# ecmwf/anemoi-core

Measured on AMD Instinct MI355X. Metric: forward nodes*channels/sec on O96 GraphTransformer, higher is better.
Workload: dtype bf16; 1 GPU; AnemoiModelEncProcDec forward, O96 data grid (40320 nodes, 84 vars x 2 steps) -> icosphere res 5 hidden mesh (10242 nodes, 81840 edges), GraphTransformer processor 16 layers x 512 ch x 16 heads, enc 62912 / dec 120960 edges, batch 1; parallelism=single GPU, hip_graph=True, graph_equals_eager=True, graph_segments=1

## Files before the change

### anemoi_core_amd/_lib.py

```python
from __future__ import annotations

import ctypes as C
import os
import threading

ABI_VERSION = 26
LIB_PATH = os.path.join(os.path.dirname(os.path.abspath(__file__)), "lib", "libanemoi_hip.so")

F32, BF16, F16 = 0, 1, 2
ACT_NONE, ACT_GELU = 0, 1
E_INVALID, E_UNSUPPORTED, E_LAUNCH = -1, -2, -3

_p, _i64, _i32, _f = C.c_void_p, C.c_int64, C.c_int32, C.c_float



class LinearPlan(C.Structure):
    _fields_ = [(name, _i32) for name in ("kernel", "tile_m", "tile_n", "pingpong", "stage_k", "mi", "wr", "kg", "stages", "epi", "main_rows",
                                          "tail_rows", "ln_tail_begin")]


class AttentionPlan(C.Structure):
    _fields_ = [(name, _i32) for name in ("route", "vec", "lph", "fe_pad", "kv_adjacent", "lds_bytes")] + \
               [(name, C.c_uint32) for name in ("grid_dst", "grid_src", "grid_wgrad")]
# ... 73 lines not shown
    "anemoi_glu_fwd": ([_p, _i64, _p, _i64, _i32, _i32, _i32, C.c_int, _p], C.c_int),
    "anemoi_glu_bwd": ([_p, _i64, _p, _i64, _p, _i64, _i32, _i32, _i32, C.c_int, _p], C.c_int),
    "anemoi_gather_rows": ([_p, _i64, _p, _p, _i64, _i32, _i32, C.c_int, _p], C.c_int),
    "anemoi_peer_alloc": ([C.POINTER(_p), _i64, _i32], C.c_int),
    "anemoi_peer_free": ([_p], C.c_int),
    "anemoi_peer_export": ([_p, _p], C.c_int),
    "anemoi_peer_open": ([_p, C.POINTER(_p)], C.c_int),
    "anemoi_peer_close": ([_p], C.c_int),
    "anemoi_gt_chain_rows_per_tile": ([_i32], C.c_int),
    "anemoi_chain_plan": ([C.POINTER(ChainProblem), C.POINTER(ChainPlan)], C.c_int),
    "anemoi_gt_chain2_fwd": ([_p, C.c_int, _p], C.c_int),
    "anemoi_gt_rowchain_fwd": ([_p, C.c_int, _p], C.c_int),
    "anemoi_gt_rowchain_panels_fwd": ([_p, C.c_int32, C.c_int32, C.c_int, _p], C.c_int),
    "anemoi_gt_embed_fold_fwd": ([_p, C.c_int, _p], C.c_int),
    "anemoi_gt_chain2_side_fwd": ([_p, _p, C.c_int32, C.c_int32, C.c_int32, C.c_int, _p], C.c_int),
    "anemoi_gt_cluster_chain_fwd": ([_p, C.c_int, _p], C.c_int),
    "anemoi_gt_cluster_chain_workspace_bytes": ([], _i64),
    "anemoi_gnn_edge_chain_fwd": ([_p, _i64, _p, _i64, _p, _p, _i64, _p, _p, _p, _p, _p, _p, _p, _p, _p, _f, _p, _i64, _i32, _i32, C.c_int, _p], C.c_int),
    "anemoi_gnn_mlp_chain_fwd": ([_p, _i64, _i32, _p, _p, _p, _p, _p, _p, _p, _p, _f, _p, _i64, _p, _i64, _i32, _i32, C.c_int, _p], C.c_int),
    "anemoi_gnn_node_chain_segsum_fwd": ([_p, _i64, _p, _i64, _p, _p, _p, _p, _p, _p, _p, _p, _p, _f, _p, _i64, _p, _p, _i32, _p, _i64, _i32, _i32,
                                          C.c_int, _p], C.c_int),
    "anemoi_gnn_node_chain_fwd": ([_p, _i64, _p, _i64, _p, _p, _p, _p, _p, _p, _p, _p, _f, _p, _i64, _p, _p, _i32, _p, _i64, _i32, _i32, C.c_int, _p], C.c_int),
    "anemoi_peer_exchange_rows": ([_p, _i64, _p, _p, _i32, _i32, _i32, _p, _p, _i64, _p], C.c_int),
    "anemoi_window_attention_fwd": ([_p, _i64, _p, _i64, _p, _i64, _p, _i64, _p, _i32, _i32, _i32, _i32, _i32, _f, _f, _p, C.c_int, _p], C.c_int),
    "anemoi_window_attention_bwd": ([_p, _i64, _p, _i64, _p, _i64, _p, _i64, _p, _i64, _p, _p, _i64, _p, _i64, _p, _i64, _p, _i32, _i32, _i32, _i32,
                                     _i32, _f, _f, _p, _i32, C.c_int, _p], C.c_int),
    "anemoi_window_attention_plan": ([_i32, _i32, _i32, _i32, C.c_int, _i32, _i32, C.POINTER(WindowAttentionPlan), C.POINTER(_i32), _i32], C.c_int),
    "anemoi_sparse_project_fwd": ([_p, _i64, _i64, _i32, _i64, _i32, _i32, _p, _p, _p, _p, _p, _p, _p, _i64, _i64, _i32, _i32, _i32, C.c_int, C.c_int, _p], C.c_int),
    "anemoi_sht_plan": ([_i32, _i32, C.POINTER(_i32), _i32, _i32, C.POINTER(ShtPlan)], C.c_int),
    "anemoi_sht_fwd": ([_p, _i64, _i64, _p, _i32, _i32, _p, _i32, _i32, _i32, _p, _p, _p, _p, _i64, _p], C.c_int),
# ... 76 lines not shown
```

### anemoi_core_amd/build.py

```python
from __future__ import annotations

import os
import shutil
import subprocess
import sys
from concurrent.futures import ThreadPoolExecutor

PKG = os.path.dirname(os.path.abspath(__file__))
REPO = os.path.dirname(PKG)
CSRC = os.path.join(PKG, "csrc")
LIBDIR = os.path.join(PKG, "lib")
LIBPATH = os.path.join(LIBDIR, "libanemoi_hip.so")
EXT_PATH = os.path.join(LIBDIR, "libanemoi_torch.so")
INCLUDE = os.path.join(REPO, "include")

SOURCES = ["lib.cpp", "gt_attention.hip", "gt_attention_bwd.hip", "rowwise.hip", "model_edge.hip", "rowwise_bwd.hip", "linear.hip", "wgrad.hip", "peer.hip", "gt_chain2.hip", "gt_chain2_side.hip", "gt_rowchain.hip", "gt_embed_fold.hip", "gt_cluster_chain.hip", "gnn_chain.hip", "window_attention.hip", "window_attention_bwd.hip", "sparse_project.hip", "sht.hip", "transport.hip", "transport_bwd.hip"]
EXPERIMENT_SOURCES = ["experiments/gt_chain.hip", "experiments/gnn_chain2.hip"]
EXP_LIBPATH = os.path.join(LIBDIR, "libanemoi_hip_exp.so")
ARCH = "gfx950"


def _hipcc() -> str:
    for cand in (os.environ.get("HIPCC"), shutil.which("hipcc"), "/opt/rocm/bin/hipcc"):
        if cand and os.path.exists(cand):
            return cand
    raise RuntimeError("hipcc not found (need ROCm >= 7.0)")


def _newer(target: str, deps: list[str]) -> bool:
    if not os.path.exists(target):
        return False
# ... 83 lines not shown
```

### anemoi_core_amd/csrc/chain_host.h

```cpp
#pragma once
#include "chain_plan.h"
#include "common.h"

namespace anemoi {

inline const ChainSwitches& chain_switches() {
  static const ChainSwitches sw = [] {
    ChainSwitches s;
    s.chain_rows = env_int(getenv("ANEMOI_CHAIN_ROWS"), 0, 0, kGnnEdgeRows);
    s.gnn_node_rows = ANEMOI_EXPERIMENT_ENV("ANEMOI_GNN_NODE_ROWS", 0, 0, kPanel);
    s.even_grid = ANEMOI_EXPERIMENT_ENV("ANEMOI_CHAIN2_EVEN_GRID", 1, 0, 1) != 0;
    s.max_grid = ANEMOI_EXPERIMENT_ENV("ANEMOI_CHAIN2_MAX_GRID", kChipCus, 8, kChipCus);
    s.timeline_built = kExperiments;
    return s;
  }();
  return sw;
}

inline int chain_refused(const char* who, const ChainProblem& q, const ChainPlan& p) {
  if (p.status != ANEMOI_OK)
    set_error("%s: %s (n_rows=%d in_features=%d hidden=%d q_out_features=%d rows_per_tile=%d dtype=%d)", who, p.why, q.n_rows, q.in_features, q.hidden,
              q.q_out_features, q.rows_per_tile, (int)q.dtype);
  return p.status;
}

inline bool al16(const void* q) { return (reinterpret_cast<uintptr_t>(q) & 15) == 0; }

#define ANEMOI_CHAIN_LAUNCH(kernel, max_lds, plan, stream, args)                                                                                     \
// ... 8 lines not shown
```

### anemoi_core_amd/csrc/chain_plan.h

```cpp
#pragma once
#include <stdint.h>

#include "anemoi_hip.h"

namespace anemoi {

constexpr int kXcds = 8, kCusPerXcd = 32;
constexpr int kChipCus = kXcds * kCusPerXcd;
constexpr int kCh = 512;
constexpr int kPanel = 48;
constexpr int kGnnEdgeRows = 64;
constexpr int kClusterSize = 4;
constexpr int kVecMaxElems = 6144;
constexpr int kVecMaxElemsTl = 5120;
constexpr int kRowChainMaxQ = 4 * kCh;
constexpr int kRowChainPipeMaxIn = 256;
constexpr int kEfRows = 80, kEfThreads = 256;
constexpr int kEfMaxIn = 256, kEfMaxQ = 2048;

constexpr int kRowBytes = kCh * 2;
constexpr int kBufBytes = kPanel * kRowBytes;
constexpr int kRedOff = 3 * kBufBytes;
constexpr int vec_off(int waves) { return kRedOff + kPanel * waves * 2 * 4; }
constexpr int kChainSmem = vec_off(8);
constexpr int kChain2Lds = vec_off(4) + kVecMaxElems * 2;
constexpr int kChain2TlLds = vec_off(4) + kVecMaxElemsTl * 2 + 8 * 48 * 8;
constexpr int kRowChainLds = vec_off(8) + (kCh + kRowChainMaxQ) * 2;
constexpr int kRowChainPipeLds = vec_off(4) + (kCh + kRowChainMaxQ) * 2;
constexpr int max_of(int a, int b) { return a > b ? a : b; }
constexpr int kChain2SideLds = max_of(kChain2Lds, max_of(kRowChainLds, kRowChainPipeLds));
constexpr int kClusterLds = vec_off(8) + (2 * kCh + 4 * kCh + kRowChainMaxQ) * 2;
constexpr int kGnnEdgeLds = 2 * kGnnEdgeRows * kRowBytes + kGnnEdgeRows * 8 * 2 * 4;
constexpr int ef_lds(int qc) { return kEfRows * 512 + kEfRows * 4 * 2 * 4 + 4 * 16 * 256 + (kCh + 3 * kCh * qc) * 4; }

struct ChainSwitches {
  int chain_rows = 0;
  int gnn_node_rows = 0;
  bool even_grid = true;
  int max_grid = kChipCus;
  bool timeline_built = false;
};

enum class ChainKind : int32_t { BlockTail = 0, BlockTailSide, ClusterTail, RowChain, RowChainPanels, EmbedFold, GnnEdge, GnnMlp, GnnNode };
enum class ChainKernel : int32_t {
  None = 0,
  Chain2Full,
  Chain2Part,
  Chain2TlFull,
  Chain2TlPart,
  Chain2Side,
  Cluster,
  RowChainSingle,
  RowChainPipe,
  EmbedFold,
  GnnEdge,
  GnnMlp,
  GnnNode,
};
constexpr const char* chain_kernel_name(ChainKernel k) {
  switch (k) {
    case ChainKernel::None: return "none";
    case ChainKernel::Chain2Full: return "gt_chain2_kernel";
    case ChainKernel::Chain2Part: return "gt_chain2_kernel<false,true>";
    case ChainKernel::Chain2TlFull: return "gt_chain2_kernel<true>";
    case ChainKernel::Chain2TlPart: return "gt_chain2_kernel<true,true>";
    case ChainKernel::Chain2Side: return "gt_chain2_kernel<false,true,true>";
    case ChainKernel::Cluster: return "gt_cluster_chain_kernel";
    case ChainKernel::RowChainSingle: return "gt_rowchain_kernel";
    case ChainKernel::RowChainPipe: return "gt_rowchain_pipe_kernel";
    case ChainKernel::EmbedFold: return "gt_embed_fold_kernel";
    case ChainKernel::GnnEdge: return "gnn_edge_chain_kernel";
    case ChainKernel::GnnMlp: return "gnn_edge_chain_kernel<true>";
    case ChainKernel::GnnNode: return "gnn_node_chain_kernel";
  }
  return "?";
}

struct ChainProblem {
  ChainKind kind = ChainKind::BlockTail;
  int n_rows = 0;
  int in_features = 0;
  int hidden = 0;
  int q_out_features = 0;
  int rows_per_tile = 0;
  anemoi_dtype_t dtype = ANEMOI_BF16;
  bool timeline = false;
  int first_panel = 0, panels = 0;
  int side_rows = 0, side_in_features = 0, side_q_out_features = 0, side_rows_per_tile = 0, side_cap = 0;
// ... 165 lines not shown
    case ChainKind::GnnMlp:
    case ChainKind::GnnNode: {
      if (!bits16) return refuse(ANEMOI_E_INVALID, "16-bit model dtypes only");
      if (q.n_rows < 0) return refuse(ANEMOI_E_INVALID, "n_rows must not be negative");
      if (q.kind == ChainKind::GnnMlp && !(q.in_features >= 128 && q.in_features <= kCh && q.in_features % 128 == 0))
        return refuse(ANEMOI_E_INVALID, "in_features is the zero-padded width: 128, 256, 384 or 512");
      if (q.n_rows == 0) return ChainPlan{};
      const bool node = q.kind == ChainKind::GnnNode;
      int rpt = gnn_rows_per_tile(q.n_rows, node ? kPanel : kGnnEdgeRows, sw.chain_rows);
      if (node && sw.gnn_node_rows > 0) rpt = sw.gnn_node_rows;
      set_panels(p, q.n_rows, rpt, -1);
      p.kernel = node ? ChainKernel::GnnNode : q.kind == ChainKind::GnnMlp ? ChainKernel::GnnMlp : ChainKernel::GnnEdge;
      p.lds_bytes = node ? kChainSmem : kGnnEdgeLds;
      return p;
    }
  }
  return refuse(ANEMOI_E_INVALID, "unknown kind");
}

}
```

### anemoi_core_amd/csrc/gt_chain2.hip

```cpp
#include <type_traits>

#include "rowchain_core.h"

namespace anemoi {

struct Chain2Args {
  const void* attn;  int64_t ld_attn;
  const void* xres;  int64_t ld_x;
  const char* wp;
  const char* w1;    int hc;
  const char* w2;
  const char* wq;    int qc;
  int qn;
  int q_cols;
  const void* vec;
  float eps1, epsq;
  const void* extra; int64_t ld_extra;
  void* xout;        int64_t ld_out;
  void* qout;        int64_t ld_q;
  int n_rows, rows_per_tile, n_tiles;
  int prio_a;
  int prio_q;
  int dbg;
  int warm;
// ... 368 lines not shown
  return check_launch("gt_chain2_kernel<side>");
}

#endif

}

using namespace anemoi;

#ifndef ANEMOI_CHAIN2_SIDE_TU

extern "C" int anemoi_gt_chain_rows_per_tile(int32_t) { return tail_rows_per_tile(chain_switches()); }

extern "C" int anemoi_chain_plan(const anemoi_chain_problem_t* q, anemoi_chain_plan_t* out) {
  ANEMOI_REQUIRE(q != nullptr && out != nullptr, "chain_plan: null problem or out");
  ANEMOI_REQUIRE(q->kind >= (int)ChainKind::BlockTail && q->kind <= (int)ChainKind::GnnNode, "chain_plan: unknown kind %d", q->kind);
  ChainProblem c;
  c.kind = (ChainKind)q->kind;
  c.n_rows = q->n_rows, c.in_features = q->in_features, c.hidden = q->hidden, c.q_out_features = q->q_out_features, c.rows_per_tile = q->rows_per_tile;
  c.dtype = (anemoi_dtype_t)q->dtype, c.timeline = q->timeline != 0, c.first_panel = q->first_panel, c.panels = q->panels;
  c.side_rows = q->side_rows, c.side_in_features = q->side_in_features, c.side_q_out_features = q->side_q_out_features;
  c.side_rows_per_tile = q->side_rows_per_tile, c.side_cap = q->side_cap;
  const ChainPlan p = plan_chain(c, chain_switches());
  if (p.status != ANEMOI_OK) return chain_refused("chain_plan", c, p);
  *out = anemoi_chain_plan_t{(int32_t)p.kernel, p.rows_per_panel, p.panels, p.grid, p.grid ? p.threads : 0, p.lds_bytes, p.rounds, p.idle_cus,
                             p.host_grid,       p.riders,         p.first,  p.end,  p.side_pipelined,         p.job_panels, p.pipelined, p.n_rows, p.row_begin};
  return ANEMOI_OK;
}

#endif
static ChainProblem chain2_problem(const anemoi_gt_chain2_args_t* p, anemoi_dtype_t dtype) {
// ... 87 lines not shown
```

### anemoi_core_amd/ops.py

```python
from __future__ import annotations

from dataclasses import dataclass
import functools
from typing import NamedTuple, Optional

import os

import torch
from torch import Tensor

from . import _ext, _lib

_DT = {torch.float32: _lib.F32, torch.bfloat16: _lib.BF16, torch.float16: _lib.F16}


def _dt(t: Tensor) -> int:
    try:
        return _DT[t.dtype]
    except KeyError:
        raise ValueError(f"unsupported dtype {t.dtype}; supported: float32, bfloat16, float16") from None


try:
    _raw_stream = torch._C._cuda_getCurrentRawStream
# ... 973 lines not shown
def linear_plan(role: str, n_rows: int, K: int, O: int, *, K2: int = 0, residual: bool = False, gather: bool = False, gelu: bool = False,
                dtype: torch.dtype = torch.bfloat16) -> Optional[GemmPlan]:
    out = _lib.LinearPlan()
    bits = (1 if residual else 0) | (2 if gather else 0) | (4 if gelu else 0)
    code = {torch.float32: _lib.F32, torch.bfloat16: _lib.BF16, torch.float16: _lib.F16}[dtype]
    rc = _lib.load().anemoi_linear_plan(GEMM_ROLES.index(role), n_rows, O, K, K2, bits, code, out)
    if rc == _lib.E_UNSUPPORTED:
        return None
    _lib.check(rc, "linear_plan")
    f = {name: getattr(out, name) for name, _ in out._fields_}
    return GemmPlan(**{**f, "kernel": GEMM_KERNELS[out.kernel], "pingpong": bool(out.pingpong)})


CHAIN_CHANNELS = 512

CHAIN_KINDS = ("block_tail", "block_tail_side", "cluster_tail", "row_chain", "row_chain_panels", "embed_fold", "gnn_edge", "gnn_mlp", "gnn_node")
CHAIN_KERNELS = ("none", "gt_chain2_kernel", "gt_chain2_kernel<false,true>", "gt_chain2_kernel<true>", "gt_chain2_kernel<true,true>",
                 "gt_chain2_kernel<false,true,true>", "gt_cluster_chain_kernel", "gt_rowchain_kernel", "gt_rowchain_pipe_kernel", "gt_embed_fold_kernel",
                 "gnn_edge_chain_kernel", "gnn_edge_chain_kernel<true>", "gnn_node_chain_kernel")


class ChainSideShape(NamedTuple):
    rows: int
    in_features: int
    q_out: int
    first_panel: int = 0
    panels: int = 0
    cap: int = 0
    rows_per_tile: int = 0


class ChainPlan(NamedTuple):
    kernel: str
    rows_per_panel: int
# ... 91 lines not shown
    _dev(attn, x_res, wp, w1g, w2, vec, extra, wqg)
    N, D = attn.shape
    dt = attn.dtype
    if D != CHAIN_CHANNELS or dt not in (torch.bfloat16, torch.float16):
        raise NotImplementedError(f"gt_layer_chain2: {D} channels / {dt} (built for {CHAIN_CHANNELS} channels, 16-bit dtypes)")
    if chain_plan("block_tail", N, hidden=hidden, q_out=q_out_features, rows_per_tile=int(rows_per_tile), dtype=dt, timeline=timeline is not None) is None:
        raise NotImplementedError(f"gt_layer_chain2: hidden={hidden} + q_out={q_out_features} exceed the kernel's LDS vector region")
    if tuple(x_res.shape) != (N, D) or (extra is not None and tuple(extra.shape) != (N, D)):
        raise ValueError("gt_layer_chain2: attn, x_res and extra must have the same [N, channels] shape")
    if extra is not None and not want_x_out:
        raise ValueError("gt_layer_chain2: a second residual needs x_out")
    _check_chain_images("gt_layer_chain2", dt, (("wp", wp, D * D), ("w1g", w1g, hidden * D), ("w2", w2, D * hidden), ("wqg", wqg, q_out_features * D)),
                        vec, 2 * D + hidden + q_out_features, "cat[bp, d1, b2, dq]")
    if not want_x_out and not q_out_features:
        raise ValueError("gt_layer_chain2: want_x_out=False needs a trailing projection")
    x_out = torch.empty((N, D), dtype=dt, device=attn.device) if want_x_out else None
    q_out = torch.empty((N, q_out_features), dtype=dt, device=attn.device) if q_out_features else None
    (ap, lda), (xp, ldx), (ep, lde) = _rows(attn, "attn", dt), _rows(x_res, "x_res", dt), _rows(extra, "extra", dt)
    a = _Chain2Args(ap, lda, xp, ldx, wp.data_ptr(), w1g.data_ptr(), hidden, w2.data_ptr(), 0 if wqg is None else wqg.data_ptr(), q_out_features,
                    vec.data_ptr(), float(ln1_eps), float(lnq_eps), ep, lde, 0 if x_out is None else x_out.data_ptr(), D, 0 if q_out is None else q_out.data_ptr(),
                    q_out_features, N, D, int(rows_per_tile), 0 if timeline is None else timeline.data_ptr())
    if side is None:
        _lib.check(_lib.load().anemoi_gt_chain2_fwd(_lib.C.byref(a), _dt(attn), _stream()), "gt_chain2_fwd")
    else:
        if side.x.dtype != dt or side.x.device != attn.device:
            raise ValueError("gt_layer_chain2: the side job's rows must have the tail's dtype and device")
        n_panels = side.n_panels
        count = n_panels - side.first_panel if side.panels is None else side.panels
        if not (0 <= side.first_panel and 0 <= count and side.first_panel + count <= n_panels and side.max_riders >= 0):
            raise ValueError(f"gt_layer_chain2: side panels [{side.first_panel}, +{count}) of {n_panels}, max_riders={side.max_riders}")
        b = _row_chain_args(side.x, side.we, side.wqg, side.vec, side.q_out_features, side.ln_eps, side.y, side.q, 0)
        _lib.check(_lib.load().anemoi_gt_chain2_side_fwd(_lib.C.byref(a), _lib.C.byref(b), side.first_panel, count, side.max_riders, _dt(attn),
                                                         _stream()), "gt_chain2_side_fwd")
    return x_out if q_out is None else (x_out, q_out)


def chain_idle_cus(n_rows: int) -> int:
    return chain_plan("block_tail", n_rows, hidden=CHAIN_CHANNELS).idle_cus if n_rows > 0 else 0


def row_chain_panels(n_rows: int, in_features: int, q_out: int) -> int:
    return chain_plan("row_chain", n_rows, in_features=in_features, q_out=q_out).panels


@dataclass
class ChainSide:
    x: Tensor
    we: Tensor
# ... 1012 lines not shown
```

### include/anemoi_hip.h

```cpp
#ifndef ANEMOI_HIP_H
#define ANEMOI_HIP_H

#include <stdint.h>

#ifdef __cplusplus
extern "C" {
#endif

#define ANEMOI_HIP_ABI_VERSION 26

typedef enum { ANEMOI_F32 = 0, ANEMOI_BF16 = 1, ANEMOI_F16 = 2 } anemoi_dtype_t;
typedef enum { ANEMOI_ACT_NONE = 0, ANEMOI_ACT_GELU = 1 } anemoi_act_t;

#define ANEMOI_OK 0
#define ANEMOI_E_INVALID (-1)
#define ANEMOI_E_UNSUPPORTED (-2)
#define ANEMOI_E_LAUNCH (-3)

int anemoi_hip_abi_version(void);
const char* anemoi_hip_last_error(void);

int anemoi_gt_attention_fwd(const void* q, int64_t ldq, const void* k, int64_t ldk, const void* v, int64_t ldv,
                            const void* e, int64_t lde, const int32_t* row, const int32_t* colptr,
                            const void* addend, int64_t ldadd, void* out, int64_t ldo, float* lse,
// ... 225 lines not shown

int anemoi_gt_chain2_side_fwd(const anemoi_gt_chain2_args_t* args, const anemoi_gt_rowchain_args_t* side, int32_t side_first_panel,
                              int32_t side_panels, int32_t side_blocks, anemoi_dtype_t dtype, void* stream);

typedef struct anemoi_chain_problem {
  int32_t kind, n_rows, in_features, hidden, q_out_features, rows_per_tile, dtype, timeline, first_panel, panels;
  int32_t side_rows, side_in_features, side_q_out_features, side_rows_per_tile, side_cap;
} anemoi_chain_problem_t;
typedef struct anemoi_chain_plan {
  int32_t kernel, rows_per_panel, panels, grid, threads, lds_bytes, rounds, idle_cus;
  int32_t host_grid, riders, first, end, side_pipelined;
  int32_t job_panels, pipelined, n_rows;
  int64_t row_begin;
} anemoi_chain_plan_t;
int anemoi_chain_plan(const anemoi_chain_problem_t* problem, anemoi_chain_plan_t* out);

typedef struct anemoi_gt_cluster_chain_args {
  const void* attn;   int64_t ld_attn;
  const void* x_res;  int64_t ld_x;
  const void* wp;
  const void* w1;     int32_t hidden;
  const void* w2;
  const void* wq;     int32_t q_out_features;
  const void* vec;
  float ln1_eps;      float lnq_eps;
  const void* extra;  int64_t ld_extra;
  void* x_out;        int64_t ld_out;
  void* q_out;        int64_t ld_q;
  void* ln_out;       int64_t ld_ln;
  void* q_out2;       int64_t ld_q2;      int32_t q_split;
// ... 111 lines not shown
```

Before: 9.010 billion nodes*channels/s.

## Add tall 80-row panel kernel for GraphTransformer block tail with cost-model dispatch

Adds a new fused block-tail kernel that processes 80-row panels in five 16-row bands. It streams weight fragments through a register ring and reuses each fragment across all bands, covering the projection, residual, LayerNorm, the MLP in 256-column hidden chunks, and an optional narrow q projection. A host-side cost model compares round counts, using per-round microsecond constants, against the existing 48-row chain kernel and dispatches to the tall kernel when it predicts fewer total microseconds. The aim is to cut weight-load traffic per row and the number of rounds on the processor's 10242-row layers. The trade-offs are more LDS use and reliance on hand-tuned constants.

```diff
diff --git a/anemoi_core_amd/_lib.py b/anemoi_core_amd/_lib.py
--- a/anemoi_core_amd/_lib.py
+++ b/anemoi_core_amd/_lib.py
@@ -4,7 +4,7 @@
 import os
 import threading
 
-ABI_VERSION = 26
+ABI_VERSION = 27
 LIB_PATH = os.path.join(os.path.dirname(os.path.abspath(__file__)), "lib", "libanemoi_hip.so")
 
 F32, BF16, F16 = 0, 1, 2
@@ -111,6 +111,8 @@
     "anemoi_gt_rowchain_panels_fwd": ([_p, C.c_int32, C.c_int32, C.c_int, _p], C.c_int),
     "anemoi_gt_embed_fold_fwd": ([_p, C.c_int, _p], C.c_int),
     "anemoi_gt_chain2_side_fwd": ([_p, _p, C.c_int32, C.c_int32, C.c_int32, C.c_int, _p], C.c_int),
+    "anemoi_gt_tall_tail_fwd": ([_p, C.c_int32, C.c_int, _p], C.c_int),
+    "anemoi_gt_tall_tail_pays": ([C.c_int32, C.c_int32, C.c_int32, C.c_int], C.c_int),
     "anemoi_gt_cluster_chain_fwd": ([_p, C.c_int, _p], C.c_int),
     "anemoi_gt_cluster_chain_workspace_bytes": ([], _i64),
     "anemoi_gnn_edge_chain_fwd": ([_p, _i64, _p, _i64, _p, _p, _i64, _p, _p, _p, _p, _p, _p, _p, _p, _p, _f, _p, _i64, _i32, _i32, C.c_int, _p], C.c_int),
diff --git a/anemoi_core_amd/build.py b/anemoi_core_amd/build.py
--- a/anemoi_core_amd/build.py
+++ b/anemoi_core_amd/build.py
@@ -14,7 +14,7 @@
 EXT_PATH = os.path.join(LIBDIR, "libanemoi_torch.so")
 INCLUDE = os.path.join(REPO, "include")
 
-SOURCES = ["lib.cpp", "gt_attention.hip", "gt_attention_bwd.hip", "rowwise.hip", "model_edge.hip", "rowwise_bwd.hip", "linear.hip", "wgrad.hip", "peer.hip", "gt_chain2.hip", "gt_chain2_side.hip", "gt_rowchain.hip", "gt_embed_fold.hip", "gt_cluster_chain.hip", "gnn_chain.hip", "window_attention.hip", "window_attention_bwd.hip", "sparse_project.hip", "sht.hip", "transport.hip", "transport_bwd.hip"]
+SOURCES = ["lib.cpp", "gt_attention.hip", "gt_attention_bwd.hip", "rowwise.hip", "model_edge.hip", "rowwise_bwd.hip", "linear.hip", "wgrad.hip", "peer.hip", "gt_chain2.hip", "gt_chain2_side.hip", "gt_chain2_tall.hip", "gt_rowchain.hip", "gt_embed_fold.hip", "gt_cluster_chain.hip", "gnn_chain.hip", "window_attention.hip", "window_attention_bwd.hip", "sparse_project.hip", "sht.hip", "transport.hip", "transport_bwd.hip"]
 EXPERIMENT_SOURCES = ["experiments/gt_chain.hip", "experiments/gnn_chain2.hip"]
 EXP_LIBPATH = os.path.join(LIBDIR, "libanemoi_hip_exp.so")
 ARCH = "gfx950"
diff --git a/anemoi_core_amd/csrc/chain_host.h b/anemoi_core_amd/csrc/chain_host.h
--- a/anemoi_core_amd/csrc/chain_host.h
+++ b/anemoi_core_amd/csrc/chain_host.h
@@ -12,6 +12,7 @@
     s.even_grid = ANEMOI_EXPERIMENT_ENV("ANEMOI_CHAIN2_EVEN_GRID", 1, 0, 1) != 0;
     s.max_grid = ANEMOI_EXPERIMENT_ENV("ANEMOI_CHAIN2_MAX_GRID", kChipCus, 8, kChipCus);
     s.timeline_built = kExperiments;
+    s.tall_tail = env_int(getenv("ANEMOI_TALL_TAIL"), 1, 0, 1) != 0;
     return s;
   }();
   return sw;
diff --git a/anemoi_core_amd/csrc/chain_plan.h b/anemoi_core_amd/csrc/chain_plan.h
--- a/anemoi_core_amd/csrc/chain_plan.h
+++ b/anemoi_core_amd/csrc/chain_plan.h
@@ -17,6 +17,12 @@
 constexpr int kRowChainPipeMaxIn = 256;
 constexpr int kEfRows = 80, kEfThreads = 256;
 constexpr int kEfMaxIn = 256, kEfMaxQ = 2048;
+constexpr int kTallBands = 5;
+constexpr int kTallRows = 16 * kTallBands;
+constexpr int kTallChunk = 256;
+constexpr int kTallVecMaxElems = 3584;
+constexpr int kTail48RoundUs = 72;
+constexpr int kTallRoundUs = 110;
 
 constexpr int kRowBytes = kCh * 2;
 constexpr int kBufBytes = kPanel * kRowBytes;
@@ -31,6 +37,8 @@
 constexpr int kChain2SideLds = max_of(kChain2Lds, max_of(kRowChainLds, kRowChainPipeLds));
 constexpr int kClusterLds = vec_off(8) + (2 * kCh + 4 * kCh + kRowChainMaxQ) * 2;
 constexpr int kGnnEdgeLds = 2 * kGnnEdgeRows * kRowBytes + kGnnEdgeRows * 8 * 2 * 4;
+constexpr int tall_lds(int bands) { return bands * 16 * kRowBytes + bands * 16 * kTallChunk * 2 + bands * 16 * 8 * 2 * 4 + kTallVecMaxElems * 2; }
+constexpr int kTallLds = tall_lds(kTallBands);
 constexpr int ef_lds(int qc) { return kEfRows * 512 + kEfRows * 4 * 2 * 4 + 4 * 16 * 256 + (kCh + 3 * kCh * qc) * 4; }
 
 struct ChainSwitches {
@@ -39,9 +47,10 @@
   bool even_grid = true;
   int max_grid = kChipCus;
   bool timeline_built = false;
+  bool tall_tail = true;
 };
 
-enum class ChainKind : int32_t { BlockTail = 0, BlockTailSide, ClusterTail, RowChain, RowChainPanels, EmbedFold, GnnEdge, GnnMlp, GnnNode };
+enum class ChainKind : int32_t { BlockTail = 0, BlockTailSide, ClusterTail, RowChain, RowChainPanels, EmbedFold, GnnEdge, GnnMlp, GnnNode, TallTail };
 enum class ChainKernel : int32_t {
   None = 0,
   Chain2Full,
@@ -56,6 +65,7 @@
   GnnEdge,
   GnnMlp,
   GnnNode,
+  Chain2Tall,
 };
 constexpr const char* chain_kernel_name(ChainKernel k) {
   switch (k) {
@@ -72,6 +82,7 @@
     case ChainKernel::GnnEdge: return "gnn_edge_chain_kernel";
     case ChainKernel::GnnMlp: return "gnn_edge_chain_kernel<true>";
     case ChainKernel::GnnNode: return "gnn_node_chain_kernel";
+    case ChainKernel::Chain2Tall: return "gt_chain2_tall_kernel";
   }
   return "?";
 }
@@ -267,8 +278,35 @@
       p.lds_bytes = node ? kChainSmem : kGnnEdgeLds;
       return p;
     }
+    case ChainKind::TallTail: {
+      if (!bits16) return refuse(ANEMOI_E_INVALID, "16-bit model dtypes only");
+      if (q.n_rows < 0) return refuse(ANEMOI_E_INVALID, "n_rows must not be negative");
+      if (q.timeline) return refuse(ANEMOI_E_UNSUPPORTED, "the tall tail has no in-kernel timeline");
+      if (!(q.hidden > 0 && q.hidden % kCh == 0)) return refuse(ANEMOI_E_INVALID, "hidden must be a multiple of 512");
+      if (!(q.q_out_features >= 0 && q.q_out_features < kCh && q.q_out_features % 128 == 0))
+        return refuse(ANEMOI_E_UNSUPPORTED, "the tall tail takes a narrow trailing projection (128, 256 or 384 columns) or none");
+      if (2 * kCh + q.hidden + q.q_out_features > kTallVecMaxElems) return refuse(ANEMOI_E_UNSUPPORTED, "the per-column vectors must fit their LDS region");
+      const int rpt = q.rows_per_tile > 0 ? q.rows_per_tile : kTallRows;
+      if (rpt > kTallRows) return refuse(ANEMOI_E_INVALID, "rows_per_tile exceeds the 80-row panel");
+      if (q.n_rows == 0) return ChainPlan{};
+      set_panels(p, q.n_rows, rpt, even_rounds_grid(ceil_div(q.n_rows, rpt)));
+      p.kernel = ChainKernel::Chain2Tall;
+      p.lds_bytes = kTallLds;
+      return p;
+    }
   }
   return refuse(ANEMOI_E_INVALID, "unknown kind");
 }
 
-}
+inline bool tall_tail_pays(ChainProblem q, const ChainSwitches& sw) {
+  if (!sw.tall_tail) return false;
+  q.rows_per_tile = 0, q.timeline = false;
+  q.kind = ChainKind::TallTail;
+  const ChainPlan tall = plan_chain(q, sw);
+  q.kind = ChainKind::BlockTail;
+  const ChainPlan low = plan_chain(q, sw);
+  if (tall.status != ANEMOI_OK || low.status != ANEMOI_OK || tall.kernel == ChainKernel::None || low.kernel == ChainKernel::None) return false;
+  return (int64_t)tall.rounds * kTallRoundUs < (int64_t)low.rounds * kTail48RoundUs;
+}
+
+}
diff --git a/anemoi_core_amd/csrc/gt_chain2.hip b/anemoi_core_amd/csrc/gt_chain2.hip
--- a/anemoi_core_amd/csrc/gt_chain2.hip
+++ b/anemoi_core_amd/csrc/gt_chain2.hip
@@ -406,7 +406,7 @@
 
 extern "C" int anemoi_chain_plan(const anemoi_chain_problem_t* q, anemoi_chain_plan_t* out) {
   ANEMOI_REQUIRE(q != nullptr && out != nullptr, "chain_plan: null problem or out");
-  ANEMOI_REQUIRE(q->kind >= (int)ChainKind::BlockTail && q->kind <= (int)ChainKind::GnnNode, "chain_plan: unknown kind %d", q->kind);
+  ANEMOI_REQUIRE(q->kind >= (int)ChainKind::BlockTail && q->kind <= (int)ChainKind::TallTail, "chain_plan: unknown kind %d", q->kind);
   ChainProblem c;
   c.kind = (ChainKind)q->kind;
   c.n_rows = q->n_rows, c.in_features = q->in_features, c.hidden = q->hidden, c.q_out_features = q->q_out_features, c.rows_per_tile = q->rows_per_tile;
diff --git a/anemoi_core_amd/csrc/gt_chain2_tall.hip b/anemoi_core_amd/csrc/gt_chain2_tall.hip
--- /dev/null
+++ b/anemoi_core_amd/csrc/gt_chain2_tall.hip
@@ -0,0 +1,375 @@
+#include "chain_core.h"
+
+namespace anemoi {
+
+struct TallArgs {
+  const void* attn;  int64_t ld_attn;
+  const void* xres;  int64_t ld_x;
+  const char* wp;
+  const char* w1;    int nc;
+  const char* w2;    int64_t s2;
+  const char* wq;    int qn;
+  const void* vec;   int n_vec16;
+  int hidden;
+  float eps1, epsq;
+  void* xout;        int64_t ld_out;
+  void* qout;        int64_t ld_q;
+  int n_rows, rows_per_tile, n_tiles;
+};
+
+constexpr int kTallHRow = kTallChunk * 2;
+template <int NB>
+struct TallLds {
+  static constexpr int kRows = 16 * NB;
+  static constexpr int kH = kRows * kRowBytes;
+  static constexpr int kRed = kH + kRows * kTallHRow;
+  static constexpr int kVec = kRed + kRows * 8 * 2 * 4;
+  static constexpr int kBytes = kVec + kTallVecMaxElems * 2;
+};
+static_assert(TallLds<kTallBands>::kBytes == kTallLds && TallLds<kTallBands>::kBytes == tall_lds(kTallBands), "chain_plan.h prices this layout");
+static_assert(kTallLds <= 160 * 1024, "LDS budget");
+static_assert(kTallVecMaxElems / 8 <= 512, "one 16-byte piece of the vectors per thread");
+
+__device__ __forceinline__ const char* tall_frag(const char* base, int i, int sh) { return base + (i >> sh) * 4096 + (i & ((1 << sh) - 1)) * 1024; }
+
+__device__ __forceinline__ void tall_ring_head(frag8 (&ring)[16], const char* base, int sh, uint32_t loff) {
+#pragma unroll
+  for (int s = 0; s < 16; ++s) {
+    ring[s] = *reinterpret_cast<gfrag_t>(uniform_ptr(tall_frag(base, s, sh)) + loff);
+    __builtin_amdgcn_sched_barrier(0);
+  }
+}
+
+template <typename T, int NB, int NI, int KS, int ROWB>
+__device__ __forceinline__ void tall_gemm(const unsigned char* abuf, int lane, frag8 (&ring)[16], const char* cur, const char* nxt, int nsh,
+                                          uint32_t loff, f32x4 (&acc)[NB][NI]) {
+  static_assert(NI == 1 || NI == 2 || NI == 4, "a K-step's fragments divide the ring");
+  constexpr int G = 16 / NI, NG = KS / G;
+  static_assert(KS % G == 0, "whole turns of the ring");
+  asm volatile("" : "+v"(lane));
+  const int x = lane & 15, ks = lane >> 4;
+  const unsigned char* arow = abuf + x * ROWB;
+  frag8 fa[NB];
+#pragma unroll
+  for (int mi = 0; mi < NB; ++mi) fa[mi] = *reinterpret_cast<const frag8*>(arow + mi * 16 * ROWB + ((ks ^ x) << 4));
+#pragma unroll 1
+  for (int q = 0; q < NG; ++q) {
+    const bool last = q == NG - 1;
+    const char* const ahead = cur + (q + 1) * G * 4096;
+#pragma unroll
+    for (int j = 0; j < G; ++j) {
+      const int st = q * G + j;
+      const int sn = st < KS - 1 ? st + 1 : KS - 1;
+      frag8 fn[NB];
+#pragma unroll
+      for (int mi = 0; mi < NB; ++mi) fn[mi] = *reinterpret_cast<const frag8*>(arow + mi * 16 * ROWB + (((sn * 4 + ks) ^ x) << 4));
+      __builtin_amdgcn_sched_barrier(0);
+#pragma unroll
+      for (int ni = 0; ni < NI; ++ni) {
+        const int slot = j * NI + ni;
+#pragma unroll
+        for (int mi = 0; mi < NB; ++mi) acc[mi][ni] = mfma16<T>(ring[slot], fa[mi], acc[mi][ni]);
+        const char* const p = last ? tall_frag(nxt, slot, nsh) : ahead + j * 4096 + ni * 1024;
+        ring[slot] = *reinterpret_cast<gfrag_t>(uniform_ptr(p) + loff);
+        __builtin_amdgcn_sched_barrier(0);
+      }
+#pragma unroll
+      for (int mi = 0; mi < NB; ++mi) fa[mi] = fn[mi];
+      __builtin_amdgcn_sched_barrier(0);
+    }
+  }
+}
+
+template <typename T, int NB>
+__device__ __forceinline__ void tall_request_rows(const T* src, int64_t ld, int r0, int nr, int lane, int w, u32x4 (&v)[2 * NB]) {
+#pragma unroll
+  for (int i = 0; i < 2 * NB; ++i) {
+    const int row = w * (2 * NB) + i;
+    v[i] = stream_load(reinterpret_cast<const u32x4*>(src + (int64_t)(r0 + min(row, nr - 1)) * ld + lane * 8));
+  }
+}
+template <int NB>
+__device__ __forceinline__ void tall_put_rows(const u32x4 (&v)[2 * NB], int nr, unsigned char* panel, int lane, int w) {
+  asm volatile("" : "+v"(lane), "+s"(w));
+#pragma unroll
+  for (int i = 0; i < 2 * NB; ++i) {
+    const int row = w * (2 * NB) + i;
+    *reinterpret_cast<u32x4*>(panel_at(panel, row, lane)) = row < nr ? v[i] : u32x4{0u, 0u, 0u, 0u};
+  }
+}
+
+template <typename T, int NB>
+__global__ __launch_bounds__(512, 1) void gt_chain2_tall_kernel(TallArgs a) {
+  using L = TallLds<NB>;
+  constexpr int R = L::kRows;
+  extern __shared__ __attribute__((aligned(16))) unsigned char smem[];
+  unsigned char* const panel = smem;
+  unsigned char* const hbuf = smem + L::kH;
+  float* const red = reinterpret_cast<float*>(smem + L::kRed);
+  const unsigned char* const vec = smem + L::kVec;
+  const int tid = threadIdx.x, lane = tid & 63;
+  const int w = __builtin_amdgcn_readfirstlane(tid >> 6);
+  const uint32_t loff = lane * 16;
+  if ((int)blockIdx.x >= a.n_tiles) return;
+  const int nc = a.nc, qn = a.qn;
+  const char* const wpw = a.wp + (int64_t)w * kSlab;
+  auto w1c = [&](int c) { return a.w1 + (int64_t)(4 * c + (w >> 1)) * kSlab + (w & 1) * 2048; };
+  auto w2c = [&](int c) { return a.w2 + (int64_t)w * a.s2 + (int64_t)c * (kTallChunk / 32) * 4096; };
+  auto wqp = [&](int p) { return a.wq + (int64_t)(2 * p + (w >> 2)) * kSlab + (w & 3) * 1024; };
+  if (tid < a.n_vec16) reinterpret_cast<u32x4*>(smem + L::kVec)[tid] = reinterpret_cast<const u32x4*>(a.vec)[tid];
+  frag8 ring[16];
+  f32x4 acc[NB][4];
+  bool first = true;
+  for (int tile = blockIdx.x; tile < a.n_tiles; tile += (int)gridDim.x) {
+    const int r0 = tile * a.rows_per_tile;
+    const int nr = min(a.rows_per_tile, a.n_rows - r0);
+    u32x4 xv[2 * NB];
+    {
+      u32x4 av[2 * NB];
+      tall_request_rows<T, NB>((const T*)a.attn, a.ld_attn, r0, nr, lane, w, av);
+      __builtin_amdgcn_sched_barrier(0);
+      tall_request_rows<T, NB>((const T*)a.xres, a.ld_x, r0, nr, lane, w, xv);
+      __builtin_amdgcn_sched_barrier(0);
+      if (first) tall_ring_head(ring, wpw, 2, loff);
+      first = false;
+      tall_put_rows<NB>(av, nr, panel, lane, w);
+    }
+    lds_barrier();
+#pragma unroll
+    for (int mi = 0; mi < NB; ++mi)
+#pragma unroll
+      for (int ni = 0; ni < 4; ++ni) acc[mi][ni] = f32x4{0.f, 0.f, 0.f, 0.f};
+    tall_gemm<T, NB, 4, 16, kRowBytes>(panel, lane, ring, wpw, w1c(0), 1, loff, acc);
+    lds_barrier();
+    tall_put_rows<NB>(xv, nr, panel, lane, w);
+    lds_barrier();
+    {
+      const LaneCols<4> lc = lane_cols<4>(lane, w);
+#pragma unroll
+      for (int mi = 0; mi < NB; ++mi) {
+        const unsigned char* prow = panel + (mi * 16 + lc.x) * kRowBytes;
+#pragma unroll
+        for (int ni = 0; ni < 4; ++ni) {
+          float b[4], r[4], o[4];
+          unpack4<T>(*reinterpret_cast<const u32x2*>(vec + (w * 64 + ni * 16 + lc.g * 4) * 2), b);
+          unpack4<T>(*reinterpret_cast<const u32x2*>(prow + lc.coff[ni]), r);
+#pragma unroll
+          for (int k = 0; k < 4; ++k) o[k] = acc[mi][ni][k] + (b[k] + r[k]);
+          unpack4<T>(pack4<T>(o), o);
+          acc[mi][ni] = f32x4{o[0], o[1], o[2], o[3]};
+        }
+        const float2 p = row_partial<4>(acc[mi]);
+        if (lc.g == 0) *reinterpret_cast<float2*>(red + ((mi * 16 + lc.x) * 8 + w) * 2) = p;
+      }
+    }
+    lds_barrier();
+    {
+      const LaneCols<4> lc = lane_cols<4>(lane, w);
+#pragma unroll
+      for (int mi = 0; mi < NB; ++mi) {
+        float mu, rstd;
+        merge_partials<8>(red, mi * 16 + lc.x, a.eps1, mu, rstd);
+        const float nm = -mu * rstd;
+        unsigned char* prow = panel + (mi * 16 + lc.x) * kRowBytes;
+#pragma unroll
+        for (int ni = 0; ni < 4; ++ni) {
+          float o[4], b[4];
+#pragma unroll
+          for (int k = 0; k < 4; ++k) o[k] = fmaf(acc[mi][ni][k], rstd, nm);
+          *reinterpret_cast<u32x2*>(prow + lc.coff[ni]) = pack4<T>(o);
+          unpack4<T>(*reinterpret_cast<const u32x2*>(vec + (kCh + a.hidden + w * 64 + ni * 16 + lc.g * 4) * 2), b);
+          acc[mi][ni] = f32x4{b[0] + acc[mi][ni][0], b[1] + acc[mi][ni][1], b[2] + acc[mi][ni][2], b[3] + acc[mi][ni][3]};
+        }
+      }
+    }
+    lds_barrier();
+#pragma unroll 1
+    for (int c = 0; c < nc; ++c) {
+      f32x4 acc1[NB][2];
+      {
+        int l1 = lane;
+        asm volatile("" : "+v"(l1));
+        const int g = l1 >> 4;
+#pragma unroll
+        for (int ni = 0; ni < 2; ++ni) {
+          float b[4];
+          unpack4<T>(*reinterpret_cast<const u32x2*>(vec + (kCh + c * kTallChunk + w * 32 + ni * 16 + g * 4) * 2), b);
+#pragma unroll
+          for (int mi = 0; mi < NB; ++mi) acc1[mi][ni] = f32x4{b[0], b[1], b[2], b[3]};
+        }
+      }
+      tall_gemm<T, NB, 2, 16, kRowBytes>(panel, lane, ring, w1c(c), w2c(c), 2, loff, acc1);
+      lds_barrier();
+      {
+        int l1 = lane;
+        asm volatile("" : "+v"(l1));
+        const int x = l1 & 15, g = l1 >> 4;
+#pragma unroll
+        for (int mi = 0; mi < NB; ++mi) {
+          unsigned char* hrow = hbuf + (mi * 16 + x) * kTallHRow;
+#pragma unroll
+          for (int ni = 0; ni < 2; ++ni) {
+            float o[4] = {acc1[mi][ni][0], acc1[mi][ni][1], acc1[mi][ni][2], acc1[mi][ni][3]};
+            gelu_fast2(o[0], o[1]);
+            gelu_fast2(o[2], o[3]);
+            *reinterpret_cast<u32x2*>(hrow + (((w * 4 + ni * 2 + (g >> 1)) ^ x) << 4) + (g & 1) * 8) = pack4<T>(o);
+            __builtin_amdgcn_sched_barrier(0);
+          }
+        }
+      }
+      lds_barrier();
+      const bool more = c + 1 < nc;
+      tall_gemm<T, NB, 4, kTallChunk / 32, kTallHRow>(hbuf, lane, ring, w2c(c), more ? w1c(c + 1) : (qn > 0 ? wqp(0) : wpw), more ? 1 : (qn > 0 ? 0 : 2),
+                                                     loff, acc);
+    }
+    {
+      const LaneCols<4> lc = lane_cols<4>(lane, w);
+#pragma unroll
+      for (int mi = 0; mi < NB; ++mi) {
+        unsigned char* prow = panel + (mi * 16 + lc.x) * kRowBytes;
+#pragma unroll
+        for (int ni = 0; ni < 4; ++ni) {
+          float o[4] = {acc[mi][ni][0], acc[mi][ni][1], acc[mi][ni][2], acc[mi][ni][3]};
+          const u32x2 pk = pack4<T>(o);
+          if (a.xout != nullptr) *reinterpret_cast<u32x2*>(prow + lc.coff[ni]) = pk;
+          unpack4<T>(pk, o);
+          acc[mi][ni] = f32x4{o[0], o[1], o[2], o[3]};
+        }
+        if (qn > 0) {
+          const float2 p = row_partial<4>(acc[mi]);
+          if (lc.g == 0) *reinterpret_cast<float2*>(red + ((mi * 16 + lc.x) * 8 + w) * 2) = p;
+        }
+      }
+    }
+    lds_barrier();
+    if (a.xout != nullptr) {
+      int l0 = lane, w0 = w;
+      asm volatile("" : "+v"(l0), "+s"(w0));
+#pragma unroll
+      for (int i = 0; i < 2 * NB; ++i) {
+        const int row = w0 * (2 * NB) + i;
+        const u32x4 v = *reinterpret_cast<const u32x4*>(panel_at(panel, row, l0));
+        if (row < nr) stream_store(v, reinterpret_cast<u32x4*>((T*)a.xout + (int64_t)(r0 + row) * a.ld_out + l0 * 8));
+      }
+      lds_barrier();
+    }
+    if (qn > 0) {
+      {
+        const LaneCols<4> lc = lane_cols<4>(lane, w);
+#pragma unroll
+        for (int mi = 0; mi < NB; ++mi) {
+          float mu, rstd;
+          merge_partials<8>(red, mi * 16 + lc.x, a.epsq, mu, rstd);
+          const float nm = -mu * rstd;
+          unsigned char* prow = panel + (mi * 16 + lc.x) * kRowBytes;
+#pragma unroll
+          for (int ni = 0; ni < 4; ++ni) {
+            float o[4];
+#pragma unroll
+            for (int k = 0; k < 4; ++k) o[k] = fmaf(acc[mi][ni][k], rstd, nm);
+            *reinterpret_cast<u32x2*>(prow + lc.coff[ni]) = pack4<T>(o);
+          }
+        }
+      }
+      lds_barrier();
+#pragma unroll 1
+      for (int p = 0; p < qn; ++p) {
+        f32x4 accq[NB][1];
+        int l1 = lane;
+        asm volatile("" : "+v"(l1));
+        const int x = l1 & 15, g = l1 >> 4;
+        {
+          float b[4];
+          unpack4<T>(*reinterpret_cast<const u32x2*>(vec + (2 * kCh + a.hidden + p * 128 + w * 16 + g * 4) * 2), b);
+#pragma unroll
+          for (int mi = 0; mi < NB; ++mi) accq[mi][0] = f32x4{b[0], b[1], b[2], b[3]};
+        }
+        const bool more = p + 1 < qn;
+        tall_gemm<T, NB, 1, 16, kRowBytes>(panel, lane, ring, wqp(p), more ? wqp(p + 1) : wpw, more ? 0 : 2, loff, accq);
+#pragma unroll
+        for (int mi = 0; mi < NB; ++mi) {
+          const float o[4] = {accq[mi][0][0], accq[mi][0][1], accq[mi][0][2], accq[mi][0][3]};
+          *reinterpret_cast<u32x2*>(hbuf + (mi * 16 + x) * kTallHRow + (((w * 2 + (g >> 1)) ^ x) << 4) + (g & 1) * 8) = pack4<T>(o);
+        }
+        lds_barrier();
+        {
+          int t0 = tid;
+          asm volatile("" : "+v"(t0));
+#pragma unroll
+          for (int it = 0; it < (R * 16 + 511) / 512; ++it) {
+            const int idx = it * 512 + t0, row = idx >> 4, s = idx & 15;
+            if (row < nr) {
+              const u32x4 v = *reinterpret_cast<const u32x4*>(hbuf + row * kTallHRow + ((s ^ (row & 15)) << 4));
+              stream_store(v, reinterpret_cast<u32x4*>((T*)a.qout + (int64_t)(r0 + row) * a.ld_q + p * 128 + s * 8));
+            }
+          }
+        }
+        lds_barrier();
+      }
+    }
+  }
+}
+
+template <typename T>
+static int launch_tall(const TallArgs& a, const ChainPlan& plan, hipStream_t st) {
+  ANEMOI_CHAIN_LAUNCH((gt_chain2_tall_kernel<T, kTallBands>), kTallLds, plan, st, a);
+  return check_launch("gt_chain2_tall_kernel");
+}
+
+}
+
+using namespace anemoi;
+
+static ChainProblem tall_problem(const anemoi_gt_chain2_args_t* p, anemoi_dtype_t dtype) {
+  ChainProblem q;
+  q.kind = ChainKind::TallTail;
+  q.n_rows = p->n_rows, q.hidden = p->hidden, q.q_out_features = p->q_out_features, q.rows_per_tile = p->rows_per_tile, q.dtype = dtype;
+  q.timeline = p->timeline != nullptr;
+  return q;
+}
+
+extern "C" int anemoi_gt_tall_tail_pays(int32_t n_rows, int32_t hidden, int32_t q_out_features, anemoi_dtype_t dtype) {
+  ChainProblem q;
+  q.n_rows = n_rows, q.hidden = hidden, q.q_out_features = q_out_features, q.dtype = dtype;
+  return tall_tail_pays(q, chain_switches()) ? 1 : 0;
+}
+
+extern "C" int anemoi_gt_tall_tail_fwd(const anemoi_gt_chain2_args_t* p, int32_t max_workgroups, anemoi_dtype_t dtype, void* stream) {
+  const char* who = "gt_tall_tail_fwd";
+  ANEMOI_REQUIRE(p != nullptr, "%s: null argument block", who);
+  ANEMOI_REQUIRE(p->channels == kCh, "%s: channels=%d (this kernel is built for %d)", who, p->channels, kCh);
+  ANEMOI_REQUIRE(max_workgroups >= 0, "%s: max_workgroups must not be negative", who);
+  const ChainProblem q = tall_problem(p, dtype);
+  ChainPlan plan = plan_chain(q, chain_switches());
+  if (plan.status == ANEMOI_OK && p->extra != nullptr) plan = refuse(ANEMOI_E_UNSUPPORTED, "the tall tail takes no second residual");
+  if (plan.status != ANEMOI_OK) return chain_refused(who, q, plan);
+  if (plan.grid == 0) return ANEMOI_OK;
+  ANEMOI_REQUIRE(p->attn && p->x_res && p->wp && p->w1 && p->w2 && p->vec && (p->x_out || p->q_out_features > 0), "%s: null operand", who);
+  ANEMOI_REQUIRE(p->q_out_features == 0 || (p->wq && p->q_out), "%s: the trailing projection needs wq and q_out", who);
+  ANEMOI_REQUIRE(al16(p->attn) && al16(p->x_res) && al16(p->wp) && al16(p->w1) && al16(p->w2) && al16(p->x_out) && al16(p->wq) && al16(p->q_out) && al16(p->vec),
+                 "%s: operands must be 16-byte aligned", who);
+  ANEMOI_REQUIRE(p->ld_attn >= kCh && p->ld_x >= kCh && p->ld_attn % 8 == 0 && p->ld_x % 8 == 0 && (p->x_out == nullptr || (p->ld_out >= kCh && p->ld_out % 8 == 0)) &&
+                     (p->q_out_features == 0 || (p->ld_q >= p->q_out_features && p->ld_q % 8 == 0)),
+                 "%s: leading dimensions too small or not multiples of 8 elements (rows move as 16-byte pieces)", who);
+  if (max_workgroups > 0 && max_workgroups < plan.grid) {
+    plan.grid = max_workgroups;
+    plan.rounds = ceil_div(plan.panels, plan.grid);
+  }
+  TallArgs a{};
+  a.attn = p->attn; a.ld_attn = p->ld_attn;
+  a.xres = p->x_res; a.ld_x = p->ld_x;
+  a.wp = (const char*)p->wp;
+  a.w1 = (const char*)p->w1; a.nc = p->hidden / kTallChunk;
+  a.w2 = (const char*)p->w2; a.s2 = (int64_t)(p->hidden / 32) * 4096;
+  a.wq = (const char*)p->wq; a.qn = p->q_out_features / 128;
+  a.vec = p->vec; a.n_vec16 = (2 * kCh + p->hidden + p->q_out_features) / 8;
+  a.hidden = p->hidden;
+  a.eps1 = p->ln1_eps; a.epsq = p->lnq_eps;
+  a.xout = p->x_out; a.ld_out = p->ld_out;
+  a.qout = p->q_out; a.ld_q = p->ld_q;
+  a.n_rows = p->n_rows;
+  a.rows_per_tile = plan.rows_per_panel;
+  a.n_tiles = plan.panels;
+  hipStream_t st = as_stream(stream);
+  return dtype == ANEMOI_BF16 ? launch_tall<bf16_t>(a, plan, st) : launch_tall<f16_t>(a, plan, st);
+}
diff --git a/anemoi_core_amd/ops.py b/anemoi_core_amd/ops.py
--- a/anemoi_core_amd/ops.py
+++ b/anemoi_core_amd/ops.py
@@ -1011,10 +1011,11 @@
 
 CHAIN_CHANNELS = 512
 
-CHAIN_KINDS = ("block_tail", "block_tail_side", "cluster_tail", "row_chain", "row_chain_panels", "embed_fold", "gnn_edge", "gnn_mlp", "gnn_node")
+CHAIN_KINDS = ("block_tail", "block_tail_side", "cluster_tail", "row_chain", "row_chain_panels", "embed_fold", "gnn_edge", "gnn_mlp", "gnn_node",
+               "tall_tail")
 CHAIN_KERNELS = ("none", "gt_chain2_kernel", "gt_chain2_kernel<false,true>", "gt_chain2_kernel<true>", "gt_chain2_kernel<true,true>",
                  "gt_chain2_kernel<false,true,true>", "gt_cluster_chain_kernel", "gt_rowchain_kernel", "gt_rowchain_pipe_kernel", "gt_embed_fold_kernel",
-                 "gnn_edge_chain_kernel", "gnn_edge_chain_kernel<true>", "gnn_node_chain_kernel")
+                 "gnn_edge_chain_kernel", "gnn_edge_chain_kernel<true>", "gnn_node_chain_kernel", "gt_chain2_tall_kernel")
 
 
 class ChainSideShape(NamedTuple):
@@ -1136,6 +1137,10 @@
                         vec, 2 * D + hidden + q_out_features, "cat[bp, d1, b2, dq]")
     if not want_x_out and not q_out_features:
         raise ValueError("gt_layer_chain2: want_x_out=False needs a trailing projection")
+    if (not rows_per_tile and timeline is None and side is None and extra is None and q_out_features < D
+            and gt_tall_tail_pays(attn, hidden, q_out_features)):
+        return gt_tall_tail(attn, x_res, wp, w1g, w2, vec, hidden, ln1_eps, wqg=wqg, q_out_features=q_out_features, lnq_eps=lnq_eps,
+                            want_x_out=want_x_out)
     x_out = torch.empty((N, D), dtype=dt, device=attn.device) if want_x_out else None
     q_out = torch.empty((N, q_out_features), dtype=dt, device=attn.device) if q_out_features else None
     (ap, lda), (xp, ldx), (ep, lde) = _rows(attn, "attn", dt), _rows(x_res, "x_res", dt), _rows(extra, "extra", dt)
@@ -1154,6 +1159,49 @@
         b = _row_chain_args(side.x, side.we, side.wqg, side.vec, side.q_out_features, side.ln_eps, side.y, side.q, 0)
         _lib.check(_lib.load().anemoi_gt_chain2_side_fwd(_lib.C.byref(a), _lib.C.byref(b), side.first_panel, count, side.max_riders, _dt(attn),
                                                          _stream()), "gt_chain2_side_fwd")
+    return x_out if q_out is None else (x_out, q_out)
+
+
+@functools.lru_cache(maxsize=1024)
+def _tall_tail_pays(n_rows: int, hidden: int, q_out: int, dtype: torch.dtype) -> bool:
+    code = {torch.bfloat16: _lib.BF16, torch.float16: _lib.F16}.get(dtype)
+    return code is not None and bool(_lib.load().anemoi_gt_tall_tail_pays(n_rows, hidden, q_out, code))
+
+
+def gt_tall_tail_pays(x: Tensor, hidden: int, q_out: int = 0) -> bool:
+    return x.dim() == 2 and x.shape[1] == CHAIN_CHANNELS and _tall_tail_pays(x.shape[0], int(hidden), int(q_out), x.dtype)
+
+
+def gt_tall_tail(attn: Tensor, x_res: Tensor, wp: Tensor, w1g: Tensor, w2: Tensor, vec: Tensor, hidden: int, ln1_eps: float, *,
+                 wqg: Optional[Tensor] = None, q_out_features: int = 0, lnq_eps: float = 1e-5, rows_per_tile: int = 0,
+                 max_workgroups: int = 0, want_x_out: bool = True, out: Optional[tuple[Optional[Tensor], Optional[Tensor]]] = None):
+    _dev(attn, x_res, wp, w1g, w2, vec, wqg)
+    N, D = attn.shape
+    dt = attn.dtype
+    if D != CHAIN_CHANNELS or dt not in (torch.bfloat16, torch.float16):
+        raise NotImplementedError(f"gt_tall_tail: {D} channels / {dt} (built for {CHAIN_CHANNELS} channels, 16-bit dtypes)")
+    if chain_plan("tall_tail", N, hidden=hidden, q_out=q_out_features, rows_per_tile=int(rows_per_tile), dtype=dt) is None:
+        raise NotImplementedError(f"gt_tall_tail: hidden={hidden}, q_out={q_out_features}: a narrow trailing projection whose vectors fit LDS")
+    if tuple(x_res.shape) != (N, D):
+        raise ValueError("gt_tall_tail: attn and x_res must have the same [N, channels] shape")
+    _check_chain_images("gt_tall_tail", dt, (("wp", wp, D * D), ("w1g", w1g, hidden * D), ("w2", w2, D * hidden), ("wqg", wqg, q_out_features * D)),
+                        vec, 2 * D + hidden + q_out_features, "cat[bp, d1, b2, dq]")
+    if not want_x_out and not q_out_features:
+        raise ValueError("gt_tall_tail: want_x_out=False needs a trailing projection")
+    x_out = torch.empty((N, D), dtype=dt, device=attn.device) if want_x_out else None
+    q_out = torch.empty((N, q_out_features), dtype=dt, device=attn.device) if q_out_features else None
+    if out is not None:
+        x_out, q_out = (out[0] if want_x_out else None), (out[1] if q_out_features else None)
+        for t, shape in ((x_out, (N, D)), (q_out, (N, q_out_features))):
+            if t is not None and (tuple(t.shape) != shape or t.dtype != dt or t.device != attn.device or not t.is_contiguous()):
+                raise ValueError(f"gt_tall_tail: out must hold contiguous {shape} {dt} rows on the operands' device")
+        if (want_x_out and x_out is None) or (q_out_features and q_out is None):
+            raise ValueError("gt_tall_tail: out lacks a wanted output")
+    (ap, lda), (xp, ldx) = _rows(attn, "attn", dt), _rows(x_res, "x_res", dt)
+    a = _Chain2Args(ap, lda, xp, ldx, wp.data_ptr(), w1g.data_ptr(), hidden, w2.data_ptr(), 0 if wqg is None else wqg.data_ptr(), q_out_features,
+                    vec.data_ptr(), float(ln1_eps), float(lnq_eps), 0, 0, 0 if x_out is None else x_out.data_ptr(), D, 0 if q_out is None else q_out.data_ptr(),
+                    q_out_features, N, D, int(rows_per_tile), 0)
+    _lib.check(_lib.load().anemoi_gt_tall_tail_fwd(_lib.C.byref(a), int(max_workgroups), _dt(attn), _stream()), "gt_tall_tail_fwd")
     return x_out if q_out is None else (x_out, q_out)
 
 
diff --git a/include/anemoi_hip.h b/include/anemoi_hip.h
--- a/include/anemoi_hip.h
+++ b/include/anemoi_hip.h
@@ -7,7 +7,7 @@
 extern "C" {
 #endif
 
-#define ANEMOI_HIP_ABI_VERSION 26
+#define ANEMOI_HIP_ABI_VERSION 27
 
 typedef enum { ANEMOI_F32 = 0, ANEMOI_BF16 = 1, ANEMOI_F16 = 2 } anemoi_dtype_t;
 typedef enum { ANEMOI_ACT_NONE = 0, ANEMOI_ACT_GELU = 1 } anemoi_act_t;
@@ -263,6 +263,9 @@
   int64_t row_begin;
 } anemoi_chain_plan_t;
 int anemoi_chain_plan(const anemoi_chain_problem_t* problem, anemoi_chain_plan_t* out);
+
+int anemoi_gt_tall_tail_fwd(const anemoi_gt_chain2_args_t* args, int32_t max_workgroups, anemoi_dtype_t dtype, void* stream);
+int anemoi_gt_tall_tail_pays(int32_t n_rows, int32_t hidden, int32_t q_out_features, anemoi_dtype_t dtype);
 
 typedef struct anemoi_gt_cluster_chain_args {
   const void* attn;   int64_t ld_attn;
```

Result: no change. 8.997 billion nodes*channels/s, median of 2 (-0.1%).
